# pathwaycom/pathway

Hardware: AMD Instinct MI355X
Metric: events/sec (whole node) on WordCount stream + p50 RAG query latency at fixed QPS (higher is better)
Workload: dtype int64/string-dict; 1 GPU; model=wordcount: stream -> groupby(word).count -> output deltas, global_batch=4000000, seq_len=1, parallelism=dp1 (shard exchange: RCCL all-to-all), vocab=50000, ingest=bytes, emitted_delta_rows=126750000, dict_misses=0

## Files before the change

pathway_amd/ops/__init__.py:

```python

from __future__ import annotations

import contextlib
import ctypes
import os
from typing import Sequence

import torch

_THIS = os.path.dirname(os.path.abspath(__file__))
_LIB_PATH = os.path.join(_THIS, "libpwhip.so")

_lib = None
_load_error: Exception | None = None


def _try_load():
    global _lib, _load_error
    if _lib is not None:
        return _lib
    try:
        if not os.path.exists(_LIB_PATH):
            from pathway_amd.ops import build as _build

# ... 467 lines not shown
    )
    oarr = (ctypes.c_void_p * max(nacc, 1))(
        *[ctypes.c_void_p(c.data_ptr()) for c in out_accs]
    )
    owarr = (ctypes.c_void_p * nw)(
        *[ctypes.c_void_p(w.data_ptr()) for w in out_words]
    )
    rc = lib.pw_seg_reduce_emit(
        warr,
        ctypes.c_int(nw),
        carr,
        ctypes.c_int(nacc),
        ctypes.c_int64(n),
        ctypes.c_void_p(bases.data_ptr()),
        owarr,
        ctypes.c_void_p(out_first.data_ptr()),
        oarr,
        ctypes.c_int64(nblocks),
        _stream_ptr(),
    )
    if rc != 0:
        raise RuntimeError(f"pw_seg_reduce_emit failed: hip error {rc}")
    return out_words, out_first, out_accs


def seg_reduce_gpu(
    k0: torch.Tensor, k1: torch.Tensor, contribs: Sequence[torch.Tensor]
) -> tuple[torch.Tensor, torch.Tensor, torch.Tensor, list]:
    out_words, out_first, out_accs = seg_reduce_words_gpu([k0, k1], contribs)
    return out_words[0], out_words[1], out_first, out_accs


_gc_temp_bytes: dict[int, int] = {}
_gc_temp_bytes_prefix: dict[int, int] = {}

_PW_GC_FULL_SORT = bool(os.environ.get("PW_GC_FULL_SORT"))

class _GcPathCounts(dict):

    bucket = 0

    def __getitem__(self, key):
        return self.bucket if key == "bucket" else dict.__getitem__(self, key)

    def __setitem__(self, key, value):
        if key == "bucket":
            self.bucket = value
        else:
            dict.__setitem__(self, key, value)


gc_path_counts = _GcPathCounts({"prefix": 0, "fallback": 0, "full": 0})

_gc_bucket_scope = False


@contextlib.contextmanager
def gc_bucket_scope(on: bool):
    global _gc_bucket_scope
    old, _gc_bucket_scope = _gc_bucket_scope, bool(on)
    try:
        yield
    finally:
        _gc_bucket_scope = old

gc_last_dirty_runs = 0

GC_BUCKET_MAX_LOAD = 0.5
GC_BUCKET_BITS = 8
GC_BUCKET_ROWS_FACTOR = 4
GC_BUCKET_MAX_PROBE = 128
GC_BUCKET_ROWS_FLOOR = 65536

_gc_bucket_caps: dict[int, int] = {}


def gc_bucket_capacity_limit(nacc: int) -> int:
    cap = _gc_bucket_caps.get(nacc)
    if cap is None:
        fn = require_lib().pw_gc_bucket_max_capacity
        fn.restype = ctypes.c_int64
        cap = int(fn(ctypes.c_int(nacc)))
        if cap < 2:
            raise RuntimeError("pw_gc_bucket_max_capacity failed")
        _gc_bucket_caps[nacc] = cap
    return cap


def gc_bucket_capacity(nacc: int) -> int:
    return min(gc_bucket_capacity_limit(nacc), 2048)


def gc_bucket_key_budget(nacc: int, bucket_bits: int = GC_BUCKET_BITS,
                         table_capacity: int | None = None) -> int:
    cap = table_capacity or gc_bucket_capacity(nacc)
    return (1 << bucket_bits) * int(GC_BUCKET_MAX_LOAD * cap)


def _gc_temp(lib, n: int, prefix: bool, dev) -> tuple[torch.Tensor, int]:
    cache = _gc_temp_bytes_prefix if prefix else _gc_temp_bytes
    tbytes = cache.get(n)
    if tbytes is None:
        fn = lib.pw_gc_temp_bytes_prefix if prefix else lib.pw_gc_temp_bytes
        fn.restype = ctypes.c_int64
        tbytes = int(fn(ctypes.c_int64(n)))
        if tbytes <= 0:
            raise RuntimeError("pw_gc_temp_bytes failed")
        cache[n] = tbytes
    return torch.empty(tbytes, dtype=torch.uint8, device=dev), tbytes


def _group_combine_two_sorts(keys_n2, contribs):
    k0, k1 = keys_n2[:, 0], keys_n2[:, 1]
    perm = torch.argsort(k1, stable=True)
    perm = perm.index_select(0, torch.argsort(k0.index_select(0, perm), stable=True))
    uk0, uk1, first_sorted, accs = seg_reduce_gpu(
        k0.index_select(0, perm),
        k1.index_select(0, perm),
        [c.index_select(0, perm) for c in contribs],
    )
    return uk0, uk1, perm.index_select(0, first_sorted), accs


def _group_combine_bucket(
    lib, keys_n2, contribs, bucket_bits, table_capacity, max_bucket_rows
):
    n = keys_n2.shape[0]
    dev = keys_n2.device
    nacc = len(contribs)
    nb = 1 << bucket_bits
    max_distinct = max(1, int(GC_BUCKET_MAX_LOAD * table_capacity))
    stream = _stream_ptr()
    temp, tbytes = _gc_temp(lib, n, True, dev)
    scratch32 = torch.empty((3, n), dtype=torch.int32, device=dev)
    staged = torch.empty((2 + max(nacc, 1), n), dtype=torch.int64, device=dev)
    bounds = torch.empty(2 * nb + 1, dtype=torch.int32, device=dev)
    base_ctl = torch.empty(nb + 3, dtype=torch.int64, device=dev)
    carr = (ctypes.c_void_p * max(nacc, 1))(
        *[ctypes.c_void_p(c.data_ptr()) for c in contribs]
    )
    sarr = (ctypes.c_void_p * max(nacc, 1))(
        *[ctypes.c_void_p(staged[2 + a].data_ptr()) for a in range(nacc)]
    )
    rc = lib.pw_gc_bucket_agg(
        ctypes.c_void_p(keys_n2.data_ptr()),
        ctypes.c_int64(n),
        ctypes.c_void_p(temp.data_ptr()),
        ctypes.c_int64(tbytes),
        ctypes.c_void_p(scratch32[0].data_ptr()),
        ctypes.c_void_p(scratch32[1].data_ptr()),
        ctypes.c_int(bucket_bits),
        ctypes.c_int64(table_capacity),
        ctypes.c_int64(max_distinct),
        ctypes.c_int64(max_bucket_rows),
        ctypes.c_int64(min(table_capacity, GC_BUCKET_MAX_PROBE)),
        carr,
        ctypes.c_int(nacc),
        ctypes.c_void_p(bounds.data_ptr()),
        ctypes.c_void_p(bounds[nb + 1 :].data_ptr()),
        ctypes.c_void_p(base_ctl.data_ptr()),
        ctypes.c_void_p(staged[0].data_ptr()),
        ctypes.c_void_p(staged[1].data_ptr()),
        ctypes.c_void_p(scratch32[2].data_ptr()),
        sarr,
        ctypes.c_void_p(base_ctl[nb + 1 :].data_ptr()),
        stream,
    )
    if rc != 0:
        raise RuntimeError(f"pw_gc_bucket_agg failed: hip error {rc}")
    total, overflow = base_ctl[nb + 1 :].tolist()
    if overflow:
        return None
    out_k = torch.empty((2, total), dtype=torch.int64, device=dev)
    out_first = torch.empty(total, dtype=torch.int64, device=dev)
    out_accs = torch.empty((max(nacc, 1), total), dtype=torch.int64, device=dev)
    oarr = (ctypes.c_void_p * max(nacc, 1))(
        *[ctypes.c_void_p(out_accs[a].data_ptr()) for a in range(nacc)]
    )
    rc = lib.pw_gc_bucket_compact(
        ctypes.c_void_p(base_ctl.data_ptr()),
        ctypes.c_void_p(bounds.data_ptr()),
        ctypes.c_int(bucket_bits),
        ctypes.c_int64(total),
        ctypes.c_void_p(staged[0].data_ptr()),
        ctypes.c_void_p(staged[1].data_ptr()),
        ctypes.c_void_p(scratch32[2].data_ptr()),
        sarr,
        ctypes.c_int(nacc),
        ctypes.c_void_p(out_k[0].data_ptr()),
        ctypes.c_void_p(out_k[1].data_ptr()),
        ctypes.c_void_p(out_first.data_ptr()),
        oarr,
        stream,
    )
    if rc != 0:
        raise RuntimeError(f"pw_gc_bucket_compact failed: hip error {rc}")
    return out_k[0], out_k[1], out_first, [out_accs[a] for a in range(nacc)]


def group_combine_gpu(
    keys_n2: torch.Tensor,
    contribs: Sequence[torch.Tensor],
    *,
    prefix_bits: int = 32,
    max_run: int = 2048,
    max_dirty: int = 65536,
    full_sort: bool = False,
    bucket: bool | None = None,
    bucket_bits: int = GC_BUCKET_BITS,
    table_capacity: int | None = None,
    max_bucket_rows: int | None = None,
) -> tuple[torch.Tensor, torch.Tensor, torch.Tensor, list]:
    global gc_last_dirty_runs
    lib = require_lib()
    n = keys_n2.shape[0]
    dev = keys_n2.device
    nacc = len(contribs)
    assert keys_n2.dim() == 2 and keys_n2.shape[1] == 2
    assert keys_n2.dtype == torch.int64
    assert 2 <= n < 2**32 and nacc <= 8
    assert 1 <= prefix_bits <= 32 and 2 <= max_run <= 3072
    assert 1 <= max_dirty < 2**32
    if keys_n2.stride() != (2, 1):
        keys_n2 = keys_n2.contiguous()
    contribs = [c.contiguous() for c in contribs]
    assert all(c.dtype == torch.int64 and c.shape == (n,) for c in contribs)
    if bucket is None:
        bucket = _gc_bucket_scope
    if bucket and not (full_sort or _PW_GC_FULL_SORT) and n < 2**32 - 1:
        assert 1 <= bucket_bits <= 16
        cap = table_capacity or gc_bucket_capacity(nacc)
        assert 2 <= cap <= gc_bucket_capacity_limit(nacc) and cap & (cap - 1) == 0
        if max_bucket_rows is None:
            even = -(-n // (1 << bucket_bits))
            max_bucket_rows = max(GC_BUCKET_ROWS_FACTOR * even, GC_BUCKET_ROWS_FLOOR)
        assert max_bucket_rows >= 1
        res = _group_combine_bucket(
            lib, keys_n2, contribs, bucket_bits, cap, max_bucket_rows
        )
        if res is not None:
            gc_path_counts["bucket"] += 1
            return res
    sorted_k = torch.empty((2, n), dtype=torch.int64, device=dev)
    perm32 = torch.empty(n, dtype=torch.int32, device=dev)
    nblocks = (n + 255) // 256
    block_counts = torch.empty(nblocks, dtype=torch.int32, device=dev)
    csum_ctrl = torch.empty(nblocks + 2, dtype=torch.int64, device=dev)
    csum = csum_ctrl[:nblocks]
    dirty_list = torch.empty(max_dirty, dtype=torch.int32, device=dev)
    stream = _stream_ptr()
    full_sort = full_sort or _PW_GC_FULL_SORT
    nseg = -1
    if not full_sort:
        temp, tbytes = _gc_temp(lib, n, True, dev)
        rc = lib.pw_gc_prefix_sort_count(
            ctypes.c_void_p(keys_n2.data_ptr()),
            ctypes.c_int64(n),
            ctypes.c_void_p(temp.data_ptr()),
            ctypes.c_int64(tbytes),
            ctypes.c_void_p(sorted_k[0].data_ptr()),
            ctypes.c_void_p(sorted_k[1].data_ptr()),
            ctypes.c_void_p(perm32.data_ptr()),
            ctypes.c_int(prefix_bits),
            ctypes.c_int64(max_run),
            ctypes.c_int64(max_dirty),
            ctypes.c_void_p(dirty_list.data_ptr()),
            ctypes.c_void_p(csum_ctrl[nblocks:].data_ptr()),
            ctypes.c_void_p(block_counts.data_ptr()),
            stream,
        )
        if rc != 0:
            raise RuntimeError(f"pw_gc_prefix_sort_count failed: hip error {rc}")
        torch.cumsum(block_counts, 0, dtype=torch.int64, out=csum)
        nseg, overflow, gc_last_dirty_runs = csum_ctrl[nblocks - 1 :].tolist()
        if overflow:
            nseg = -1
        else:
            gc_path_counts["prefix"] += 1
    if nseg < 0:
        temp, tbytes = _gc_temp(lib, n, False, dev)
        rc = lib.pw_gc_sort_count(
            ctypes.c_void_p(keys_n2.data_ptr()),
            ctypes.c_int64(n),
            ctypes.c_void_p(temp.data_ptr()),
            ctypes.c_int64(tbytes),
            ctypes.c_void_p(sorted_k[0].data_ptr()),
            ctypes.c_void_p(sorted_k[1].data_ptr()),
            ctypes.c_void_p(perm32.data_ptr()),
            ctypes.c_int(4),
            ctypes.c_int64(max_run),
            ctypes.c_int64(max_dirty),
            ctypes.c_void_p(dirty_list.data_ptr()),
            ctypes.c_void_p(csum_ctrl[nblocks:].data_ptr()),
            ctypes.c_void_p(block_counts.data_ptr()),
# ... 856 lines not shown
```

pathway_amd/ops/csrc/hip/pw_kernels.hip:

```cpp
#include <hip/hip_runtime.h>
#include <stdint.h>
#include <stdio.h>

#include <cstring>
#include <rocprim/rocprim.hpp>

#include "../xxhash_common.h"

#define PW_BLOCK 256
#define PW_MAX_GRID 2048

static inline int pw_grid(int64_t n) {
  int64_t g = (n + PW_BLOCK - 1) / PW_BLOCK;
  if (g > PW_MAX_GRID) g = PW_MAX_GRID;
  if (g < 1) g = 1;
  return (int)g;
}


struct WordPtrs {
  const uint64_t* p[20];
};

template <int W>
// ... 2406 lines not shown
                     s, (const long long*)keys, (const uint32_t*)perm32,
                     (long long*)k1_sorted, n, (unsigned long long*)ctrl);
  int64_t pairs = n / 2 + 1;
  int64_t rblocks = (pairs + PW_BLOCK - 1) / PW_BLOCK;
  for (int p = 0; p < passes; ++p)
    hipLaunchKernelGGL(k_gc_sort_repair, dim3((uint32_t)rblocks),
                       dim3(PW_BLOCK), 0, s, (const long long*)k0_sorted,
                       (long long*)k1_sorted, (uint32_t*)perm32, n, p & 1);
  return gc_repair_count(k0_sorted, k1_sorted, perm32, n, 0, max_run,
                         max_dirty, dirty_list, ctrl, block_counts, s);
}

extern "C" int64_t pw_gc_temp_bytes_prefix(int64_t n) {
  size_t bytes = 0;
  if (n <= 0 || n >= ((int64_t)1 << 32)) return 0;
  if (gc_sort_prefix(nullptr, bytes, nullptr, nullptr, nullptr, n, 32, 0) !=
      hipSuccess)
    return 0;
  return (int64_t)bytes;
}

extern "C" int pw_gc_prefix_sort_count(const void* keys, int64_t n, void* temp,
                                       int64_t temp_bytes, void* k0_sorted,
                                       void* k1_sorted, void* perm32,
                                       int prefix_bits, int64_t max_run,
                                       int64_t max_dirty, void* dirty_list,
                                       void* ctrl, void* block_counts,
                                       void* stream) {
  if (n < 2 || n >= ((int64_t)1 << 32)) return 1;
  if (prefix_bits < 1 || prefix_bits > 32) return 1;
  if (max_run < 2 || max_run > PW_GC_MAX_RUN_LIMIT) return 1;
  if (max_dirty < 1 || max_dirty >= ((int64_t)1 << 32)) return 1;
  hipStream_t s = (hipStream_t)stream;
  size_t tb = (size_t)temp_bytes;
  hipError_t e = gc_sort_prefix(temp, tb, (const long long*)keys,
                                (uint32_t*)k1_sorted, (uint32_t*)perm32, n,
                                prefix_bits, s);
  if (e != hipSuccess) return (int)e;
  hipLaunchKernelGGL(k_gc_gather_k01, dim3(2 * PW_MAX_GRID), dim3(PW_BLOCK), 0,
                     s, (const long long*)keys, (const uint32_t*)perm32,
                     (long long*)k0_sorted, (long long*)k1_sorted, n,
                     (unsigned long long*)ctrl);
  return gc_repair_count(k0_sorted, k1_sorted, perm32, n, 64 - prefix_bits,
                         max_run, max_dirty, dirty_list, ctrl, block_counts,
                         s);
}


#define PW_GC_BK_THREADS 1024
#define PW_GC_BK_UNPUB 0xFFFFFFFFu
#define PW_GC_BK_LDS_MAX 61440
#define PW_GC_BK_UNROLL 4

__global__ void k_gc_bucket_bounds(const uint32_t* __restrict__ prefix_sorted,
                                   int64_t n, uint32_t nb,
                                   uint32_t* bucket_start,
                                   unsigned long long* ctl) {
  uint32_t b = blockIdx.x * blockDim.x + threadIdx.x;
  if (b == 0) {
    ctl[0] = 0;
    ctl[1] = 0;
  }
  if (b > nb) return;
  int64_t lo = 0, hi = n;
  while (lo < hi) {
    int64_t mid = (lo + hi) >> 1;
    if (prefix_sorted[mid] < b) lo = mid + 1;
    else hi = mid;
  }
  bucket_start[b] = (uint32_t)lo;
}

__device__ __forceinline__ uint32_t gc_bk_hash(unsigned long long w0,
                                               long long w1, int lg_cap) {
  uint32_t h = (uint32_t)w0 ^ (uint32_t)(w0 >> 29) ^
               ((uint32_t)w1 * 0x9E3779B1u);
  return (h * 0x85EBCA6Bu) >> (32 - lg_cap);
}

__global__ __launch_bounds__(PW_GC_BK_THREADS) void k_gc_bucket_agg(
    const long long* __restrict__ keys, const uint32_t* __restrict__ perm32,
    const uint32_t* __restrict__ bucket_start, AccPtrs contribs, int nacc,
    int bucket_bits, uint32_t cap, int lg_cap, uint32_t max_distinct,
    uint32_t max_rows, uint32_t max_probe, long long* st_k0, long long* st_k1,
    uint32_t* st_first, AccPtrsMut st_accs, uint32_t* bucket_uniques,
    unsigned long long* ctl) {
  extern __shared__ unsigned long long gcb_lds[];
  unsigned long long* t0 = gcb_lds;
  long long* t1 = (long long*)(t0 + cap);
  unsigned long long* tacc = (unsigned long long*)(t1 + cap);
  uint32_t* tfirst = (uint32_t*)(tacc + (size_t)nacc * cap);
  uint16_t* list = (uint16_t*)(tfirst + cap);
  __shared__ uint32_t s_cnt, s_claims, s_ovf;

  const uint32_t b = blockIdx.x;
  const uint32_t tid = threadIdx.x;
  const uint32_t beg = bucket_start[b], end = bucket_start[b + 1];
  const uint32_t rows = end - beg;
  if (rows == 0 || rows > max_rows) {
    if (tid == 0) {
      bucket_uniques[b] = 0;
      if (rows) ctl[1] = 1;
    }
    return;
  }
  const uint32_t mask = cap - 1;
  const unsigned long long empty =
      (unsigned long long)((b ^ 1u) ^ (1u << (bucket_bits - 1)))
      << (64 - bucket_bits);
  for (uint32_t s = tid; s < cap; s += PW_GC_BK_THREADS) {
    t0[s] = empty;
    tfirst[s] = PW_GC_BK_UNPUB;
    for (int a = 0; a < nacc; ++a) tacc[(size_t)a * cap + s] = 0;
  }
  if (tid == 0) s_cnt = 0, s_claims = 0, s_ovf = 0;
  __syncthreads();

  const long long* c0 = contribs.p[0];
  for (int64_t base = (int64_t)beg + tid; base < (int64_t)end;
       base += (int64_t)PW_GC_BK_UNROLL * PW_GC_BK_THREADS) {
    uint32_t row[PW_GC_BK_UNROLL];
    unsigned long long k0[PW_GC_BK_UNROLL];
    long long k1[PW_GC_BK_UNROLL];
    unsigned long long v0[PW_GC_BK_UNROLL];
#pragma unroll
    for (int q = 0; q < PW_GC_BK_UNROLL; ++q) {
      int64_t i = base + (int64_t)q * PW_GC_BK_THREADS;
      row[q] = i < (int64_t)end ? perm32[i] : PW_GC_BK_UNPUB;
    }
#pragma unroll
    for (int q = 0; q < PW_GC_BK_UNROLL; ++q) {
      if (row[q] == PW_GC_BK_UNPUB) continue;
      k0[q] = (unsigned long long)keys[2 * (size_t)row[q]];
      k1[q] = keys[2 * (size_t)row[q] + 1];
      v0[q] = nacc > 0 ? (unsigned long long)c0[row[q]] : 0ULL;
    }
#pragma unroll
    for (int q = 0; q < PW_GC_BK_UNROLL; ++q) {
      if (row[q] == PW_GC_BK_UNPUB) continue;
      if (__hip_atomic_load(&s_ovf, __ATOMIC_RELAXED,
                            __HIP_MEMORY_SCOPE_WORKGROUP))
        break;
      const unsigned long long key0 = k0[q];
      const long long key1 = k1[q];
      uint32_t slot = gc_bk_hash(key0, key1, lg_cap);
      bool done = false;
      for (uint32_t tries = 0; tries < max_probe; ++tries) {
        bool match;
        const unsigned long long cur = __hip_atomic_load(
            &t0[slot], __ATOMIC_ACQUIRE, __HIP_MEMORY_SCOPE_WORKGROUP);
        if (cur != empty) {
          match = cur == key0 && t1[slot] == key1;
          if (match) atomicMin(&tfirst[slot], row[q]);
        } else {
          const uint32_t f = atomicCAS(&tfirst[slot], PW_GC_BK_UNPUB, row[q]);
          match = f == PW_GC_BK_UNPUB;
          if (match) {
            if (atomicAdd(&s_claims, 1u) >= max_distinct) s_ovf = 1;
            t1[slot] = key1;
            __hip_atomic_store(&t0[slot], key0, __ATOMIC_RELEASE,
                               __HIP_MEMORY_SCOPE_WORKGROUP);
          } else {
            match = (unsigned long long)keys[2 * (size_t)f] == key0 &&
                    keys[2 * (size_t)f + 1] == key1;
            if (match) atomicMin(&tfirst[slot], row[q]);
          }
        }
        if (match) {
          if (nacc > 0) atomicAdd(&tacc[slot], v0[q]);
          for (int a = 1; a < nacc; ++a)
            atomicAdd(&tacc[(size_t)a * cap + slot],
                      (unsigned long long)contribs.p[a][row[q]]);
          done = true;
          break;
        }
        slot = (slot + 1) & mask;
      }
      if (!done) s_ovf = 1;
    }
  }
  __syncthreads();

  for (uint32_t s = tid; s < cap; s += PW_GC_BK_THREADS)
    if (tfirst[s] != PW_GC_BK_UNPUB) list[atomicAdd(&s_cnt, 1u)] = (uint16_t)s;
  __syncthreads();
  const uint32_t cnt = s_cnt;
  if (s_ovf || cnt > max_distinct) {
    if (tid == 0) {
      bucket_uniques[b] = 0;
      ctl[1] = 1;
    }
    return;
  }

  for (uint32_t t = tid; t < cnt; t += PW_GC_BK_THREADS) {
    const uint32_t sl = list[t];
    const long long a0 = (long long)t0[sl], a1 = t1[sl];
    uint32_t rank = 0;
    for (uint32_t u = 0; u < cnt; ++u) {
      const uint32_t su = list[u];
      const long long b0 = (long long)t0[su];
      rank += (b0 < a0 || (b0 == a0 && t1[su] < a1)) ? 1u : 0u;
    }
    const size_t o = (size_t)beg + rank;
    st_k0[o] = a0;
    st_k1[o] = a1;
    st_first[o] = tfirst[sl];
    for (int a = 0; a < nacc; ++a)
      st_accs.p[a][o] = (long long)tacc[(size_t)a * cap + sl];
  }
  if (tid == 0) bucket_uniques[b] = cnt;
}

__global__ void k_gc_bucket_scan(const uint32_t* __restrict__ uniq,
                                 uint32_t nb, long long* base,
                                 unsigned long long* ctl) {
  __shared__ long long part[PW_BLOCK];
  const uint32_t tid = threadIdx.x;
  const uint32_t chunk = (nb + PW_BLOCK - 1) / PW_BLOCK;
  const uint32_t lo = tid * chunk < nb ? tid * chunk : nb;
  const uint32_t hi = lo + chunk < nb ? lo + chunk : nb;
  long long sum = 0;
  for (uint32_t i = lo; i < hi; ++i) sum += uniq[i];
  part[tid] = sum;
  __syncthreads();
// ... 42 lines not shown
static inline size_t gc_bk_entry_bytes(int nacc) {
  return 8 + 8 + 8 * (size_t)nacc + 4 + 2;
}

extern "C" int64_t pw_gc_bucket_max_capacity(int nacc) {
  if (nacc < 0 || nacc > 8) return 0;
  int64_t cap = 1;
  while ((size_t)(2 * cap) * gc_bk_entry_bytes(nacc) <= PW_GC_BK_LDS_MAX)
    cap *= 2;
  return cap;
}

extern "C" int pw_gc_bucket_agg(const void* keys, int64_t n, void* temp,
                                int64_t temp_bytes, void* prefix_scratch,
                                void* perm32, int bucket_bits,
                                int64_t table_capacity, int64_t max_distinct,
                                int64_t max_bucket_rows, int64_t max_probe,
                                const void** contrib_ptrs, int nacc,
                                void* bucket_start, void* bucket_uniques,
                                void* base, void* st_k0, void* st_k1,
                                void* st_first, void** st_acc_ptrs, void* ctl,
                                void* stream) {
  if (n < 2 || n >= ((int64_t)1 << 32) - 1) return 1;
  if (bucket_bits < 1 || bucket_bits > 16) return 1;
  if (nacc < 0 || nacc > 8) return 1;
  if (table_capacity < 2 || table_capacity > 32768 ||
      (table_capacity & (table_capacity - 1)))
    return 1;
  size_t lds = (size_t)table_capacity * gc_bk_entry_bytes(nacc);
  if (lds > PW_GC_BK_LDS_MAX) return 1;
  if (max_distinct < 1 || max_distinct > table_capacity) return 1;
  if (max_bucket_rows < 1 || max_probe < 1) return 1;
  if (max_bucket_rows > 0xFFFFFFFFLL) max_bucket_rows = 0xFFFFFFFFLL;
  if (max_probe > table_capacity) max_probe = table_capacity;
  int lg_cap = 0;
  while (((int64_t)1 << lg_cap) < table_capacity) ++lg_cap;
  hipStream_t s = (hipStream_t)stream;
  size_t tb = (size_t)temp_bytes;
  hipError_t e = gc_sort_prefix(temp, tb, (const long long*)keys,
                                (uint32_t*)prefix_scratch, (uint32_t*)perm32,
                                n, bucket_bits, s);
  if (e != hipSuccess) return (int)e;
  AccPtrs cp;
  AccPtrsMut sp;
  for (int a = 0; a < 8; ++a) {
    cp.p[a] = a < nacc ? (const long long*)contrib_ptrs[a] : nullptr;
    sp.p[a] = a < nacc ? (long long*)st_acc_ptrs[a] : nullptr;
  }
  uint32_t nb = 1u << bucket_bits;
  hipLaunchKernelGGL(k_gc_bucket_bounds,
                     dim3((nb + 1 + PW_BLOCK - 1) / PW_BLOCK), dim3(PW_BLOCK),
                     0, s, (const uint32_t*)prefix_scratch, n, nb,
                     (uint32_t*)bucket_start, (unsigned long long*)ctl);
  hipLaunchKernelGGL(k_gc_bucket_agg, dim3(nb), dim3(PW_GC_BK_THREADS), lds, s,
                     (const long long*)keys, (const uint32_t*)perm32,
                     (const uint32_t*)bucket_start, cp, nacc, bucket_bits,
                     (uint32_t)table_capacity, lg_cap, (uint32_t)max_distinct,
                     (uint32_t)max_bucket_rows, (uint32_t)max_probe,
                     (long long*)st_k0, (long long*)st_k1, (uint32_t*)st_first,
                     sp, (uint32_t*)bucket_uniques, (unsigned long long*)ctl);
  hipLaunchKernelGGL(k_gc_bucket_scan, dim3(1), dim3(PW_BLOCK), 0, s,
                     (const uint32_t*)bucket_uniques, nb, (long long*)base,
                     (unsigned long long*)ctl);
  return (int)hipGetLastError();
}

extern "C" int pw_gc_bucket_compact(const void* base, const void* bucket_start,
                                    int bucket_bits, int64_t total,
                                    const void* st_k0, const void* st_k1,
                                    const void* st_first,
                                    const void** st_acc_ptrs, int nacc,
                                    void* out_k0, void* out_k1,
                                    void* out_first, void** out_acc_ptrs,
                                    void* stream) {
  if (bucket_bits < 1 || bucket_bits > 16 || nacc < 0 || nacc > 8) return 1;
  if (total < 1) return 0;
  AccPtrs sp;
  AccPtrsMut op;
  for (int a = 0; a < 8; ++a) {
    sp.p[a] = a < nacc ? (const long long*)st_acc_ptrs[a] : nullptr;
    op.p[a] = a < nacc ? (long long*)out_acc_ptrs[a] : nullptr;
  }
  int64_t nblocks = (total + PW_BLOCK - 1) / PW_BLOCK;
  hipLaunchKernelGGL(k_gc_bucket_compact, dim3((uint32_t)nblocks),
                     dim3(PW_BLOCK), 0, (hipStream_t)stream,
                     (const long long*)base, (const uint32_t*)bucket_start,
                     1u << bucket_bits, total, (const long long*)st_k0,
                     (const long long*)st_k1, (const uint32_t*)st_first, sp,
                     nacc, (long long*)out_k0, (long long*)out_k1,
                     (long long*)out_first, op);
  return (int)hipGetLastError();
}

extern "C" int pw_gc_emit(const void* k0_sorted, const void* k1_sorted,
                          const void* perm32, const void** contrib_ptrs,
                          int nacc, int64_t n, const void* block_csum,
                          void* out_k0, void* out_k1, void* out_first,
                          void** out_acc_ptrs, void* stream) {
  if (nacc < 0 || nacc > 8 || n < 1) return 1;
  AccPtrs cp;
  AccPtrsMut op;
  for (int a = 0; a < nacc; ++a) {
    cp.p[a] = (const long long*)contrib_ptrs[a];
    op.p[a] = (long long*)out_acc_ptrs[a];
  }
  hipStream_t s = (hipStream_t)stream;
  int64_t nblocks = (n + PW_BLOCK - 1) / PW_BLOCK;
  hipLaunchKernelGGL(k_gc_emit, dim3((uint32_t)nblocks), dim3(PW_BLOCK), 0, s,
                     (const long long*)k0_sorted, (const long long*)k1_sorted,
// ... 604 lines not shown
```

profiles/gc_bucket_sweep.py:

```python

import json
import statistics
import time

import torch

from pathway_amd import ops

N, VOCAB, REPS = 4_000_000, 50_000, 20


def timed(keys, contribs, **kw):
    before = {k: ops.gc_path_counts[k] for k in ("prefix", "fallback", "bucket")}
    ts = []
    for i in range(REPS + 3):
        torch.cuda.synchronize()
        t0 = time.perf_counter()
        ops.group_combine_gpu(keys, contribs, **kw)
        torch.cuda.synchronize()
        if i >= 3:
            ts.append((time.perf_counter() - t0) * 1e3)
    path = [k for k, v in before.items() if ops.gc_path_counts[k] != v]
    return round(statistics.median(ts), 4), "+".join(path)


def main():
    g = torch.Generator(device="cpu").manual_seed(1)
    table = torch.randint(-(1 << 63), (1 << 63) - 1, (VOCAB, 2), generator=g)
    keys = table[torch.randint(0, VOCAB, (N,), generator=g)].cuda()
    ones = [torch.ones(N, dtype=torch.int64, device="cuda")]
    ms, path = timed(keys, ones, bucket=False)
    print(json.dumps({"case": "50k distinct", "bucket": False, "ms": ms, "path": path}))
    for bits in (6, 8, 9, 10, 12):
        for cap in (512, 1024, 2048):
            ms, path = timed(keys, ones, bucket=True, bucket_bits=bits, table_capacity=cap)
            print(json.dumps({"case": "50k distinct", "bucket_bits": bits,
                              "table_capacity": cap, "ms": ms, "path": path}))
    distinct = torch.randint(-(1 << 63), (1 << 63) - 1, (N, 2), generator=g).cuda()
    for on in (False, True):
        ms, path = timed(distinct, ones, bucket=on)
        print(json.dumps({"case": "all distinct", "bucket": on, "ms": ms, "path": path}))


if __name__ == "__main__":
    main()
```

Baseline: 3.522 billion events/s.

## Partition rows by key bucket before hash aggregation instead of gathering via sort

Adds a three-kernel radix partition (per-tile histogram, scan, LDS-staged scatter) that physically moves keys, row ids and contributions into bucket-contiguous order, so the bucket aggregation kernel reads them with coalesced loads. Before this, the path sorted a prefix permutation and then gathered keys and contributions indirectly. The partition path becomes the default for bucket_bits <= 8. It costs extra staging memory for the partitioned copies and may clone the keys to get 16-byte alignment. It only runs when the bucket scope is enabled.

After: 3.792 billion events/s (median of 6 runs). +7.7%, better.

```diff
diff --git a/pathway_amd/ops/__init__.py b/pathway_amd/ops/__init__.py
--- a/pathway_amd/ops/__init__.py
+++ b/pathway_amd/ops/__init__.py
@@ -543,6 +543,12 @@
 
 gc_path_counts = _GcPathCounts({"prefix": 0, "fallback": 0, "full": 0})
 
+_PW_NO_GC_PARTITION = bool(os.environ.get("PW_NO_GC_PARTITION"))
+_PW_GC_PART_DIRECT = bool(os.environ.get("PW_GC_PART_DIRECT"))
+gc_bucket_layout_counts = {"partition": 0, "gather": 0}
+GC_PART_TILE = 8192
+GC_PART_MAX_BITS = 8
+
 _gc_bucket_scope = False
 
 
@@ -613,8 +619,77 @@
     return uk0, uk1, perm.index_select(0, first_sorted), accs
 
 
+def _gc_part_hist_entries(lib, n: int, bucket_bits: int) -> int:
+    fn = lib.pw_gc_part_hist_entries
+    fn.restype = ctypes.c_int64
+    entries = int(fn(ctypes.c_int64(n), ctypes.c_int(bucket_bits)))
+    if entries <= 0:
+        raise RuntimeError("pw_gc_part_hist_entries failed")
+    tile = lib.pw_gc_part_tile
+    tile.restype = ctypes.c_int64
+    assert int(tile()) == GC_PART_TILE
+    return entries
+
+
+def _gc_aligned_keys(keys_n2: torch.Tensor) -> torch.Tensor:
+    return keys_n2.clone() if keys_n2.data_ptr() % 16 else keys_n2
+
+
+def gc_partition_gpu(
+    keys_n2: torch.Tensor, contribs: Sequence[torch.Tensor], bucket_bits: int
+) -> tuple[torch.Tensor, torch.Tensor, torch.Tensor, list]:
+    lib = require_lib()
+    n = keys_n2.shape[0]
+    dev = keys_n2.device
+    nacc = len(contribs)
+    assert keys_n2.dim() == 2 and keys_n2.shape[1] == 2
+    assert keys_n2.dtype == torch.int64
+    assert 2 <= n < 2**32 - 1 and nacc <= 8 and 1 <= bucket_bits <= 8
+    if keys_n2.stride() != (2, 1):
+        keys_n2 = keys_n2.contiguous()
+    keys_n2 = _gc_aligned_keys(keys_n2)
+    contribs = [c.contiguous() for c in contribs]
+    assert all(c.dtype == torch.int64 and c.shape == (n,) for c in contribs)
+    nb = 1 << bucket_bits
+    hist = _gc_part_hist_entries(lib, n, bucket_bits)
+    part64 = torch.empty((2 + nacc, n), dtype=torch.int64, device=dev)
+    scratch32 = torch.empty(hist + n + nb + 1, dtype=torch.int32, device=dev)
+    ctl = torch.empty(2, dtype=torch.int64, device=dev)
+    carr = (ctypes.c_void_p * max(nacc, 1))(
+        *[ctypes.c_void_p(c.data_ptr()) for c in contribs]
+    )
+    parr = (ctypes.c_void_p * max(nacc, 1))(
+        *[ctypes.c_void_p(part64[2 + a].data_ptr()) for a in range(nacc)]
+    )
+    rc = lib.pw_gc_partition(
+        ctypes.c_void_p(keys_n2.data_ptr()),
+        ctypes.c_int64(n),
+        ctypes.c_int(bucket_bits),
+        carr,
+        ctypes.c_int(nacc),
+        ctypes.c_void_p(scratch32.data_ptr()),
+        ctypes.c_void_p(part64.data_ptr()),
+        ctypes.c_void_p(scratch32[hist:].data_ptr()),
+        parr,
+        ctypes.c_void_p(scratch32[hist + n :].data_ptr()),
+        ctypes.c_void_p(ctl.data_ptr()),
+        ctypes.c_int(int(_PW_GC_PART_DIRECT)),
+        _stream_ptr(),
+    )
+    if rc != 0:
+        raise RuntimeError(f"pw_gc_partition failed: hip error {rc}")
+    u32 = lambda t: t.to(torch.int64) & 0xFFFFFFFF
+    return (
+        u32(scratch32[hist + n :]),
+        part64[:2].reshape(n, 2),
+        u32(scratch32[hist : hist + n]),
+        [part64[2 + a] for a in range(nacc)],
+    )
+
+
 def _group_combine_bucket(
-    lib, keys_n2, contribs, bucket_bits, table_capacity, max_bucket_rows
+    lib, keys_n2, contribs, bucket_bits, table_capacity, max_bucket_rows,
+    partition=False,
 ):
     n = keys_n2.shape[0]
     dev = keys_n2.device
@@ -622,43 +697,86 @@
     nb = 1 << bucket_bits
     max_distinct = max(1, int(GC_BUCKET_MAX_LOAD * table_capacity))
     stream = _stream_ptr()
-    temp, tbytes = _gc_temp(lib, n, True, dev)
-    scratch32 = torch.empty((3, n), dtype=torch.int32, device=dev)
-    staged = torch.empty((2 + max(nacc, 1), n), dtype=torch.int64, device=dev)
     bounds = torch.empty(2 * nb + 1, dtype=torch.int32, device=dev)
     base_ctl = torch.empty(nb + 3, dtype=torch.int64, device=dev)
     carr = (ctypes.c_void_p * max(nacc, 1))(
         *[ctypes.c_void_p(c.data_ptr()) for c in contribs]
     )
+    if partition:
+        keys_n2 = _gc_aligned_keys(keys_n2)
+        hist = _gc_part_hist_entries(lib, n, bucket_bits)
+        scratch32 = torch.empty(hist + 2 * n, dtype=torch.int32, device=dev)
+        st_first = scratch32[hist + n :]
+        staged = torch.empty(
+            (2 + nacc + 2 + max(nacc, 1), n), dtype=torch.int64, device=dev
+        )
+        st0 = 2 + nacc
+        parr = (ctypes.c_void_p * max(nacc, 1))(
+            *[ctypes.c_void_p(staged[2 + a].data_ptr()) for a in range(nacc)]
+        )
+    else:
+        temp, tbytes = _gc_temp(lib, n, True, dev)
+        scratch32 = torch.empty((3, n), dtype=torch.int32, device=dev)
+        st_first = scratch32[2]
+        staged = torch.empty((2 + max(nacc, 1), n), dtype=torch.int64, device=dev)
+        st0 = 0
     sarr = (ctypes.c_void_p * max(nacc, 1))(
-        *[ctypes.c_void_p(staged[2 + a].data_ptr()) for a in range(nacc)]
-    )
-    rc = lib.pw_gc_bucket_agg(
-        ctypes.c_void_p(keys_n2.data_ptr()),
-        ctypes.c_int64(n),
-        ctypes.c_void_p(temp.data_ptr()),
-        ctypes.c_int64(tbytes),
-        ctypes.c_void_p(scratch32[0].data_ptr()),
-        ctypes.c_void_p(scratch32[1].data_ptr()),
-        ctypes.c_int(bucket_bits),
-        ctypes.c_int64(table_capacity),
-        ctypes.c_int64(max_distinct),
-        ctypes.c_int64(max_bucket_rows),
-        ctypes.c_int64(min(table_capacity, GC_BUCKET_MAX_PROBE)),
-        carr,
-        ctypes.c_int(nacc),
-        ctypes.c_void_p(bounds.data_ptr()),
-        ctypes.c_void_p(bounds[nb + 1 :].data_ptr()),
-        ctypes.c_void_p(base_ctl.data_ptr()),
-        ctypes.c_void_p(staged[0].data_ptr()),
-        ctypes.c_void_p(staged[1].data_ptr()),
-        ctypes.c_void_p(scratch32[2].data_ptr()),
-        sarr,
-        ctypes.c_void_p(base_ctl[nb + 1 :].data_ptr()),
-        stream,
-    )
-    if rc != 0:
-        raise RuntimeError(f"pw_gc_bucket_agg failed: hip error {rc}")
+        *[ctypes.c_void_p(staged[st0 + 2 + a].data_ptr()) for a in range(nacc)]
+    )
+    if partition:
+        rc = lib.pw_gc_bucket_part_agg(
+            ctypes.c_void_p(keys_n2.data_ptr()),
+            ctypes.c_int64(n),
+            ctypes.c_int(bucket_bits),
+            ctypes.c_int64(table_capacity),
+            ctypes.c_int64(max_distinct),
+            ctypes.c_int64(max_bucket_rows),
+            ctypes.c_int64(min(table_capacity, GC_BUCKET_MAX_PROBE)),
+            carr,
+            ctypes.c_int(nacc),
+            ctypes.c_void_p(scratch32.data_ptr()),
+            ctypes.c_void_p(staged.data_ptr()),
+            ctypes.c_void_p(scratch32[hist:].data_ptr()),
+            parr,
+            ctypes.c_void_p(bounds.data_ptr()),
+            ctypes.c_void_p(bounds[nb + 1 :].data_ptr()),
+            ctypes.c_void_p(base_ctl.data_ptr()),
+            ctypes.c_void_p(staged[st0].data_ptr()),
+            ctypes.c_void_p(staged[st0 + 1].data_ptr()),
+            ctypes.c_void_p(st_first.data_ptr()),
+            sarr,
+            ctypes.c_void_p(base_ctl[nb + 1 :].data_ptr()),
+            ctypes.c_int(int(_PW_GC_PART_DIRECT)),
+            stream,
+        )
+    else:
+        rc = lib.pw_gc_bucket_agg(
+            ctypes.c_void_p(keys_n2.data_ptr()),
+            ctypes.c_int64(n),
+            ctypes.c_void_p(temp.data_ptr()),
+            ctypes.c_int64(tbytes),
+            ctypes.c_void_p(scratch32[0].data_ptr()),
+            ctypes.c_void_p(scratch32[1].data_ptr()),
+            ctypes.c_int(bucket_bits),
+            ctypes.c_int64(table_capacity),
+            ctypes.c_int64(max_distinct),
+            ctypes.c_int64(max_bucket_rows),
+            ctypes.c_int64(min(table_capacity, GC_BUCKET_MAX_PROBE)),
+            carr,
+            ctypes.c_int(nacc),
+            ctypes.c_void_p(bounds.data_ptr()),
+            ctypes.c_void_p(bounds[nb + 1 :].data_ptr()),
+            ctypes.c_void_p(base_ctl.data_ptr()),
+            ctypes.c_void_p(staged[0].data_ptr()),
+            ctypes.c_void_p(staged[1].data_ptr()),
+            ctypes.c_void_p(st_first.data_ptr()),
+            sarr,
+            ctypes.c_void_p(base_ctl[nb + 1 :].data_ptr()),
+            stream,
+        )
+    if rc != 0:
+        fn = "pw_gc_bucket_part_agg" if partition else "pw_gc_bucket_agg"
+        raise RuntimeError(f"{fn} failed: hip error {rc}")
     total, overflow = base_ctl[nb + 1 :].tolist()
     if overflow:
         return None
@@ -673,9 +791,9 @@
         ctypes.c_void_p(bounds.data_ptr()),
         ctypes.c_int(bucket_bits),
         ctypes.c_int64(total),
-        ctypes.c_void_p(staged[0].data_ptr()),
-        ctypes.c_void_p(staged[1].data_ptr()),
-        ctypes.c_void_p(scratch32[2].data_ptr()),
+        ctypes.c_void_p(staged[st0].data_ptr()),
+        ctypes.c_void_p(staged[st0 + 1].data_ptr()),
+        ctypes.c_void_p(st_first.data_ptr()),
         sarr,
         ctypes.c_int(nacc),
         ctypes.c_void_p(out_k[0].data_ptr()),
@@ -701,6 +819,7 @@
     bucket_bits: int = GC_BUCKET_BITS,
     table_capacity: int | None = None,
     max_bucket_rows: int | None = None,
+    partition: bool | None = None,
 ) -> tuple[torch.Tensor, torch.Tensor, torch.Tensor, list]:
     global gc_last_dirty_runs
     lib = require_lib()
@@ -726,11 +845,15 @@
             even = -(-n // (1 << bucket_bits))
             max_bucket_rows = max(GC_BUCKET_ROWS_FACTOR * even, GC_BUCKET_ROWS_FLOOR)
         assert max_bucket_rows >= 1
+        if partition is None:
+            partition = not _PW_NO_GC_PARTITION
+        partition = bool(partition) and bucket_bits <= GC_PART_MAX_BITS
         res = _group_combine_bucket(
-            lib, keys_n2, contribs, bucket_bits, cap, max_bucket_rows
+            lib, keys_n2, contribs, bucket_bits, cap, max_bucket_rows, partition
         )
         if res is not None:
             gc_path_counts["bucket"] += 1
+            gc_bucket_layout_counts["partition" if partition else "gather"] += 1
             return res
     sorted_k = torch.empty((2, n), dtype=torch.int64, device=dev)
     perm32 = torch.empty(n, dtype=torch.int32, device=dev)
diff --git a/pathway_amd/ops/csrc/hip/pw_kernels.hip b/pathway_amd/ops/csrc/hip/pw_kernels.hip
--- a/pathway_amd/ops/csrc/hip/pw_kernels.hip
+++ b/pathway_amd/ops/csrc/hip/pw_kernels.hip
@@ -2482,6 +2482,243 @@
 #define PW_GC_BK_LDS_MAX 61440
 #define PW_GC_BK_UNROLL 4
 
+#define PW_GC_PT_THREADS 1024
+#define PW_GC_PT_TILE 8192
+#define PW_GC_PT_ROWS (PW_GC_PT_TILE / PW_GC_PT_THREADS)
+#define PW_GC_PT_SUB 2048
+#define PW_GC_PT_SCAN_RANGES 32
+
+__device__ __forceinline__ uint32_t gc_pt_bucket(unsigned long long w0,
+                                                 int drop) {
+  return ((uint32_t)(w0 >> 32) ^ 0x80000000u) >> drop;
+}
+
+static inline uint32_t gc_pt_stride(uint32_t nb) { return nb < 8 ? 8 : nb; }
+
+__host__ __device__ static inline uint32_t gc_pt_chunk(uint32_t nblk) {
+  return (nblk + PW_GC_PT_SCAN_RANGES - 1) / PW_GC_PT_SCAN_RANGES;
+}
+
+__global__ __launch_bounds__(PW_GC_PT_THREADS) void k_gc_part_count(
+    const long long* __restrict__ keys, int64_t n, int drop, uint32_t nbp,
+    uint32_t* __restrict__ block_hist) {
+  __shared__ uint32_t h[256];
+  const uint32_t tid = threadIdx.x;
+  if (tid < 256) h[tid] = 0;
+  __syncthreads();
+  const int64_t base = (int64_t)blockIdx.x * PW_GC_PT_TILE + tid;
+  unsigned long long w[PW_GC_PT_ROWS];
+#pragma unroll
+  for (int q = 0; q < PW_GC_PT_ROWS; ++q) {
+    const int64_t i = base + (int64_t)q * PW_GC_PT_THREADS;
+    w[q] = i < n ? (unsigned long long)keys[2 * (size_t)i] : 0ULL;
+  }
+#pragma unroll
+  for (int q = 0; q < PW_GC_PT_ROWS; ++q) {
+    const int64_t i = base + (int64_t)q * PW_GC_PT_THREADS;
+    if (i < n) atomicAdd(&h[gc_pt_bucket(w[q], drop)], 1u);
+  }
+  __syncthreads();
+  if (tid < nbp) block_hist[(size_t)blockIdx.x * nbp + tid] = h[tid];
+}
+
+__global__ __launch_bounds__(PW_GC_PT_THREADS) void k_gc_part_scan(
+    const uint32_t* __restrict__ block_hist, uint32_t nblk, uint32_t nb,
+    uint32_t nbp, int64_t n, uint32_t* __restrict__ bucket_start,
+    uint32_t* __restrict__ range_base, unsigned long long* ctl) {
+  __shared__ uint32_t part[PW_GC_PT_SCAN_RANGES][256];
+  __shared__ uint32_t sc[256];
+  const uint32_t tid = threadIdx.x;
+  const uint32_t no = nbp / 8;
+  const uint32_t tb = tid % no, tr = tid / no;
+  const bool active = tr < PW_GC_PT_SCAN_RANGES;
+  const uint32_t chunk = gc_pt_chunk(nblk);
+  const uint32_t lo = tr * chunk < nblk ? tr * chunk : nblk;
+  const uint32_t hi = lo + chunk < nblk ? lo + chunk : nblk;
+  const uint4* h4 = (const uint4*)block_hist;
+  if (tid == 0) {
+    ctl[0] = 0;
+    ctl[1] = 0;
+  }
+  if (active) {
+    uint4 s = make_uint4(0, 0, 0, 0), t = make_uint4(0, 0, 0, 0);
+#pragma unroll 8
+    for (uint32_t blk = lo; blk < hi; ++blk) {
+      const uint4 v = h4[((size_t)blk * no + tb) * 2];
+      const uint4 w = h4[((size_t)blk * no + tb) * 2 + 1];
+      s.x += v.x, s.y += v.y, s.z += v.z, s.w += v.w;
+      t.x += w.x, t.y += w.y, t.z += w.z, t.w += w.w;
+    }
+    uint32_t* p = &part[tr][8 * tb];
+    p[0] = s.x, p[1] = s.y, p[2] = s.z, p[3] = s.w;
+    p[4] = t.x, p[5] = t.y, p[6] = t.z, p[7] = t.w;
+  }
+  __syncthreads();
+  uint32_t tot = 0;
+  if (tid < nbp) {
+    for (int r = 0; r < PW_GC_PT_SCAN_RANGES; ++r) {
+      const uint32_t v = part[r][tid];
+      part[r][tid] = tot;
+      tot += v;
+    }
+  }
+  if (tid < 256) sc[tid] = tot;
+  __syncthreads();
+  for (uint32_t off = 1; off < 256; off <<= 1) {
+    const uint32_t v = (tid < 256 && tid >= off) ? sc[tid - off] : 0;
+    __syncthreads();
+    if (tid < 256) sc[tid] += v;
+    __syncthreads();
+  }
+  if (tid < 256) {
+    const uint32_t ex = sc[tid] - tot;
+    sc[tid] = ex;
+    if (tid < nb) bucket_start[tid] = ex;
+  }
+  if (tid == 0) bucket_start[nb] = (uint32_t)n;
+  __syncthreads();
+  for (uint32_t e = tid; e < PW_GC_PT_SCAN_RANGES * nbp; e += PW_GC_PT_THREADS)
+    range_base[e] = sc[e % nbp] + part[e / nbp][e % nbp];
+}
+
+template <bool STAGED>
+__global__ __launch_bounds__(PW_GC_PT_THREADS) void k_gc_part_scatter(
+    const long long* __restrict__ keys, AccPtrs contribs, int nacc, int64_t n,
+    int drop, uint32_t nbp, const uint32_t* __restrict__ block_hist,
+    const uint32_t* __restrict__ range_base, long long* __restrict__ part_keys,
+    uint32_t* __restrict__ part_row, AccPtrsMut part_acc) {
+  __shared__ uint32_t cur[256];
+  const uint32_t tid = threadIdx.x;
+  const ulonglong2* __restrict__ k2 = (const ulonglong2*)keys;
+  ulonglong2* __restrict__ o2 = (ulonglong2*)part_keys;
+  const long long* __restrict__ c0 = contribs.p[0];
+  const int64_t tile = (int64_t)blockIdx.x * PW_GC_PT_TILE;
+  if (tid < nbp) {
+    const uint32_t chunk = gc_pt_chunk(gridDim.x);
+    const uint32_t r = blockIdx.x / chunk;
+    uint32_t v = range_base[r * nbp + tid];
+    for (uint32_t blk = r * chunk; blk < blockIdx.x; ++blk)
+      v += block_hist[(size_t)blk * nbp + tid];
+    cur[tid] = v;
+  }
+  if constexpr (!STAGED) {
+    __syncthreads();
+    for (int g = 0; g < PW_GC_PT_ROWS; g += 4) {
+      ulonglong2 kv[4];
+      long long v0[4];
+#pragma unroll
+      for (int q = 0; q < 4; ++q) {
+        const int64_t i = tile + (int64_t)(g + q) * PW_GC_PT_THREADS + tid;
+        if (i < n) {
+          kv[q] = k2[i];
+          v0[q] = nacc > 0 ? c0[i] : 0;
+        }
+      }
+#pragma unroll
+      for (int q = 0; q < 4; ++q) {
+        const int64_t i = tile + (int64_t)(g + q) * PW_GC_PT_THREADS + tid;
+        if (i >= n) continue;
+        const uint32_t dst = atomicAdd(&cur[gc_pt_bucket(kv[q].x, drop)], 1u);
+        o2[dst] = kv[q];
+        part_row[dst] = (uint32_t)i;
+        if (nacc > 0) part_acc.p[0][dst] = v0[q];
+        for (int a = 1; a < nacc; ++a) part_acc.p[a][dst] = contribs.p[a][i];
+      }
+    }
+  } else {
+    constexpr int SQ = PW_GC_PT_SUB / PW_GC_PT_THREADS;
+    __shared__ ulonglong2 bufk[PW_GC_PT_SUB];
+    __shared__ long long bufa[PW_GC_PT_SUB];
+    __shared__ uint32_t bufr[PW_GC_PT_SUB];
+    __shared__ uint8_t bkt[PW_GC_PT_SUB];
+    __shared__ uint32_t cnt[256], lstart[256], delta[256], wtot[4];
+    for (int64_t sbase = tile; sbase < tile + PW_GC_PT_TILE && sbase < n;
+         sbase += PW_GC_PT_SUB) {
+      const uint32_t m =
+          n - sbase < PW_GC_PT_SUB ? (uint32_t)(n - sbase) : PW_GC_PT_SUB;
+      if (tid < 256) cnt[tid] = 0;
+      __syncthreads();
+      ulonglong2 kv[SQ];
+      long long v0[SQ];
+      uint32_t bk[SQ], lp[SQ];
+#pragma unroll
+      for (int q = 0; q < SQ; ++q) {
+        const uint32_t j = q * PW_GC_PT_THREADS + tid;
+        if (j < m) {
+          kv[q] = k2[sbase + j];
+          v0[q] = nacc > 0 ? c0[sbase + j] : 0;
+        }
+      }
+#pragma unroll
+      for (int q = 0; q < SQ; ++q) {
+        const uint32_t j = q * PW_GC_PT_THREADS + tid;
+        if (j < m) {
+          bk[q] = gc_pt_bucket(kv[q].x, drop);
+          lp[q] = atomicAdd(&cnt[bk[q]], 1u);
+        }
+      }
+      __syncthreads();
+      uint32_t c = 0, inc = 0;
+      if (tid < 256) {
+        c = cnt[tid];
+        inc = c;
+#pragma unroll
+        for (int d = 1; d < 64; d <<= 1) {
+          const uint32_t up = __shfl_up(inc, d);
+          if ((tid & 63) >= (uint32_t)d) inc += up;
+        }
+        if ((tid & 63) == 63) wtot[tid >> 6] = inc;
+      }
+      __syncthreads();
+      if (tid < 256) {
+        uint32_t off = 0;
+        for (uint32_t w = 0; w < (tid >> 6); ++w) off += wtot[w];
+        const uint32_t ex = off + inc - c;
+        lstart[tid] = ex;
+        delta[tid] = cur[tid] - ex;
+        cur[tid] += c;
+      }
+      __syncthreads();
+#pragma unroll
+      for (int q = 0; q < SQ; ++q) {
+        const uint32_t j = q * PW_GC_PT_THREADS + tid;
+        if (j < m) {
+          lp[q] += lstart[bk[q]];
+          bufk[lp[q]] = kv[q];
+          bufr[lp[q]] = (uint32_t)(sbase + j);
+          bkt[lp[q]] = (uint8_t)bk[q];
+          if (nacc > 0) bufa[lp[q]] = v0[q];
+        }
+      }
+      __syncthreads();
+#pragma unroll
+      for (int q = 0; q < SQ; ++q) {
+        const uint32_t j = q * PW_GC_PT_THREADS + tid;
+        if (j < m) {
+          const uint32_t dst = delta[bkt[j]] + j;
+          o2[dst] = bufk[j];
+          part_row[dst] = bufr[j];
+          if (nacc > 0) part_acc.p[0][dst] = bufa[j];
+        }
+      }
+      for (int a = 1; a < nacc; ++a) {
+        __syncthreads();
+#pragma unroll
+        for (int q = 0; q < SQ; ++q) {
+          const uint32_t j = q * PW_GC_PT_THREADS + tid;
+          if (j < m) bufa[lp[q]] = contribs.p[a][sbase + j];
+        }
+        __syncthreads();
+#pragma unroll
+        for (int q = 0; q < SQ; ++q) {
+          const uint32_t j = q * PW_GC_PT_THREADS + tid;
+          if (j < m) part_acc.p[a][delta[bkt[j]] + j] = bufa[j];
+        }
+      }
+    }
+  }
+}
+
 __global__ void k_gc_bucket_bounds(const uint32_t* __restrict__ prefix_sorted,
                                    int64_t n, uint32_t nb,
                                    uint32_t* bucket_start,
@@ -2508,8 +2745,10 @@
   return (h * 0x85EBCA6Bu) >> (32 - lg_cap);
 }
 
+template <bool PART, int NV>
 __global__ __launch_bounds__(PW_GC_BK_THREADS) void k_gc_bucket_agg(
     const long long* __restrict__ keys, const uint32_t* __restrict__ perm32,
+    const long long* __restrict__ part_keys,
     const uint32_t* __restrict__ bucket_start, AccPtrs contribs, int nacc,
     int bucket_bits, uint32_t cap, int lg_cap, uint32_t max_distinct,
     uint32_t max_rows, uint32_t max_probe, long long* st_k0, long long* st_k1,
@@ -2552,7 +2791,7 @@
     uint32_t row[PW_GC_BK_UNROLL];
     unsigned long long k0[PW_GC_BK_UNROLL];
     long long k1[PW_GC_BK_UNROLL];
-    unsigned long long v0[PW_GC_BK_UNROLL];
+    unsigned long long v[PW_GC_BK_UNROLL][NV];
 #pragma unroll
     for (int q = 0; q < PW_GC_BK_UNROLL; ++q) {
       int64_t i = base + (int64_t)q * PW_GC_BK_THREADS;
@@ -2561,9 +2800,19 @@
 #pragma unroll
     for (int q = 0; q < PW_GC_BK_UNROLL; ++q) {
       if (row[q] == PW_GC_BK_UNPUB) continue;
-      k0[q] = (unsigned long long)keys[2 * (size_t)row[q]];
-      k1[q] = keys[2 * (size_t)row[q] + 1];
-      v0[q] = nacc > 0 ? (unsigned long long)c0[row[q]] : 0ULL;
+      if constexpr (PART) {
+        const int64_t i = base + (int64_t)q * PW_GC_BK_THREADS;
+        const ulonglong2 kv = ((const ulonglong2*)part_keys)[i];
+        k0[q] = kv.x;
+        k1[q] = (long long)kv.y;
+#pragma unroll
+        for (int a = 0; a < NV; ++a)
+          v[q][a] = a < nacc ? (unsigned long long)contribs.p[a][i] : 0ULL;
+      } else {
+        k0[q] = (unsigned long long)keys[2 * (size_t)row[q]];
+        k1[q] = keys[2 * (size_t)row[q] + 1];
+        v[q][0] = nacc > 0 ? (unsigned long long)c0[row[q]] : 0ULL;
+      }
     }
 #pragma unroll
     for (int q = 0; q < PW_GC_BK_UNROLL; ++q) {
@@ -2597,10 +2846,16 @@
           }
         }
         if (match) {
-          if (nacc > 0) atomicAdd(&tacc[slot], v0[q]);
-          for (int a = 1; a < nacc; ++a)
-            atomicAdd(&tacc[(size_t)a * cap + slot],
-                      (unsigned long long)contribs.p[a][row[q]]);
+          if (nacc > 0) atomicAdd(&tacc[slot], v[q][0]);
+          if constexpr (PART) {
+#pragma unroll
+            for (int a = 1; a < NV; ++a)
+              if (a < nacc) atomicAdd(&tacc[(size_t)a * cap + slot], v[q][a]);
+          } else {
+            for (int a = 1; a < nacc; ++a)
+              atomicAdd(&tacc[(size_t)a * cap + slot],
+                        (unsigned long long)contribs.p[a][row[q]]);
+          }
           done = true;
           break;
         }
@@ -2749,9 +3004,127 @@
                      dim3((nb + 1 + PW_BLOCK - 1) / PW_BLOCK), dim3(PW_BLOCK),
                      0, s, (const uint32_t*)prefix_scratch, n, nb,
                      (uint32_t*)bucket_start, (unsigned long long*)ctl);
-  hipLaunchKernelGGL(k_gc_bucket_agg, dim3(nb), dim3(PW_GC_BK_THREADS), lds, s,
-                     (const long long*)keys, (const uint32_t*)perm32,
+  hipLaunchKernelGGL((k_gc_bucket_agg<false, 1>), dim3(nb),
+                     dim3(PW_GC_BK_THREADS), lds, s, (const long long*)keys,
+                     (const uint32_t*)perm32, (const long long*)nullptr,
                      (const uint32_t*)bucket_start, cp, nacc, bucket_bits,
+                     (uint32_t)table_capacity, lg_cap, (uint32_t)max_distinct,
+                     (uint32_t)max_bucket_rows, (uint32_t)max_probe,
+                     (long long*)st_k0, (long long*)st_k1, (uint32_t*)st_first,
+                     sp, (uint32_t*)bucket_uniques, (unsigned long long*)ctl);
+  hipLaunchKernelGGL(k_gc_bucket_scan, dim3(1), dim3(PW_BLOCK), 0, s,
+                     (const uint32_t*)bucket_uniques, nb, (long long*)base,
+                     (unsigned long long*)ctl);
+  return (int)hipGetLastError();
+}
+
+extern "C" int64_t pw_gc_part_tile() { return PW_GC_PT_TILE; }
+
+extern "C" int64_t pw_gc_part_hist_entries(int64_t n, int bucket_bits) {
+  if (n < 2 || n >= ((int64_t)1 << 32) - 1) return 0;
+  if (bucket_bits < 1 || bucket_bits > 8) return 0;
+  int64_t nblk = (n + PW_GC_PT_TILE - 1) / PW_GC_PT_TILE;
+  return (nblk + PW_GC_PT_SCAN_RANGES) *
+         (int64_t)gc_pt_stride(1u << bucket_bits);
+}
+
+static void gc_partition_launch(const long long* keys, int64_t n,
+                                int bucket_bits, const AccPtrs& cp, int nacc,
+                                uint32_t* block_hist, long long* part_keys,
+                                uint32_t* part_row, const AccPtrsMut& pp,
+                                uint32_t* bucket_start,
+                                unsigned long long* ctl, int direct,
+                                hipStream_t s) {
+  const uint32_t nb = 1u << bucket_bits, nbp = gc_pt_stride(nb);
+  const uint32_t nblk = (uint32_t)((n + PW_GC_PT_TILE - 1) / PW_GC_PT_TILE);
+  const int drop = 32 - bucket_bits;
+  uint32_t* range_base = block_hist + (size_t)nblk * nbp;
+  hipLaunchKernelGGL(k_gc_part_count, dim3(nblk), dim3(PW_GC_PT_THREADS), 0, s,
+                     keys, n, drop, nbp, block_hist);
+  hipLaunchKernelGGL(k_gc_part_scan, dim3(1), dim3(PW_GC_PT_THREADS), 0, s,
+                     (const uint32_t*)block_hist, nblk, nb, nbp, n,
+                     bucket_start, range_base, ctl);
+  if (direct)
+    hipLaunchKernelGGL(k_gc_part_scatter<false>, dim3(nblk),
+                       dim3(PW_GC_PT_THREADS), 0, s, keys, cp, nacc, n, drop,
+                       nbp, (const uint32_t*)block_hist,
+                       (const uint32_t*)range_base, part_keys, part_row, pp);
+  else
+    hipLaunchKernelGGL(k_gc_part_scatter<true>, dim3(nblk),
+                       dim3(PW_GC_PT_THREADS), 0, s, keys, cp, nacc, n, drop,
+                       nbp, (const uint32_t*)block_hist,
+                       (const uint32_t*)range_base, part_keys, part_row, pp);
+}
+
+static bool gc_partition_args_ok(const void* keys, int64_t n, int bucket_bits,
+                                 int nacc, const void* block_hist,
+                                 const void* part_keys) {
+  if (n < 2 || n >= ((int64_t)1 << 32) - 1) return false;
+  if (bucket_bits < 1 || bucket_bits > 8) return false;
+  if (nacc < 0 || nacc > 8) return false;
+  return ((uintptr_t)keys | (uintptr_t)block_hist | (uintptr_t)part_keys) % 16 == 0;
+}
+
+extern "C" int pw_gc_partition(const void* keys, int64_t n, int bucket_bits,
+                               const void** contrib_ptrs, int nacc,
+                               void* block_hist, void* part_keys,
+                               void* part_row, void** part_acc_ptrs,
+                               void* bucket_start, void* ctl, int direct,
+                               void* stream) {
+  if (!gc_partition_args_ok(keys, n, bucket_bits, nacc, block_hist, part_keys))
+    return 1;
+  AccPtrs cp;
+  AccPtrsMut pp;
+  for (int a = 0; a < 8; ++a) {
+    cp.p[a] = a < nacc ? (const long long*)contrib_ptrs[a] : nullptr;
+    pp.p[a] = a < nacc ? (long long*)part_acc_ptrs[a] : nullptr;
+  }
+  gc_partition_launch((const long long*)keys, n, bucket_bits, cp, nacc,
+                      (uint32_t*)block_hist, (long long*)part_keys,
+                      (uint32_t*)part_row, pp, (uint32_t*)bucket_start,
+                      (unsigned long long*)ctl, direct, (hipStream_t)stream);
+  return (int)hipGetLastError();
+}
+
+extern "C" int pw_gc_bucket_part_agg(
+    const void* keys, int64_t n, int bucket_bits, int64_t table_capacity,
+    int64_t max_distinct, int64_t max_bucket_rows, int64_t max_probe,
+    const void** contrib_ptrs, int nacc, void* block_hist, void* part_keys,
+    void* part_row, void** part_acc_ptrs, void* bucket_start,
+    void* bucket_uniques, void* base, void* st_k0, void* st_k1, void* st_first,
+    void** st_acc_ptrs, void* ctl, int direct, void* stream) {
+  if (!gc_partition_args_ok(keys, n, bucket_bits, nacc, block_hist, part_keys))
+    return 1;
+  if (table_capacity < 2 || table_capacity > 32768 ||
+      (table_capacity & (table_capacity - 1)))
+    return 1;
+  size_t lds = (size_t)table_capacity * gc_bk_entry_bytes(nacc);
+  if (lds > PW_GC_BK_LDS_MAX) return 1;
+  if (max_distinct < 1 || max_distinct > table_capacity) return 1;
+  if (max_bucket_rows < 1 || max_probe < 1) return 1;
+  if (max_bucket_rows > 0xFFFFFFFFLL) max_bucket_rows = 0xFFFFFFFFLL;
+  if (max_probe > table_capacity) max_probe = table_capacity;
+  int lg_cap = 0;
+  while (((int64_t)1 << lg_cap) < table_capacity) ++lg_cap;
+  hipStream_t s = (hipStream_t)stream;
+  AccPtrs cp, pc;
+  AccPtrsMut pp, sp;
+  for (int a = 0; a < 8; ++a) {
+    cp.p[a] = a < nacc ? (const long long*)contrib_ptrs[a] : nullptr;
+    pp.p[a] = a < nacc ? (long long*)part_acc_ptrs[a] : nullptr;
+    pc.p[a] = pp.p[a];
+    sp.p[a] = a < nacc ? (long long*)st_acc_ptrs[a] : nullptr;
+  }
+  gc_partition_launch((const long long*)keys, n, bucket_bits, cp, nacc,
+                      (uint32_t*)block_hist, (long long*)part_keys,
+                      (uint32_t*)part_row, pp, (uint32_t*)bucket_start,
+                      (unsigned long long*)ctl, direct, s);
+  const uint32_t nb = 1u << bucket_bits;
+  auto agg = nacc <= 1 ? k_gc_bucket_agg<true, 1> : k_gc_bucket_agg<true, 8>;
+  hipLaunchKernelGGL(agg, dim3(nb), dim3(PW_GC_BK_THREADS), lds, s,
+                     (const long long*)keys, (const uint32_t*)part_row,
+                     (const long long*)part_keys,
+                     (const uint32_t*)bucket_start, pc, nacc, bucket_bits,
                      (uint32_t)table_capacity, lg_cap, (uint32_t)max_distinct,
                      (uint32_t)max_bucket_rows, (uint32_t)max_probe,
                      (long long*)st_k0, (long long*)st_k1, (uint32_t*)st_first,
diff --git a/profiles/gc_bucket_sweep.py b/profiles/gc_bucket_sweep.py
--- a/profiles/gc_bucket_sweep.py
+++ b/profiles/gc_bucket_sweep.py
@@ -33,9 +33,13 @@
     print(json.dumps({"case": "50k distinct", "bucket": False, "ms": ms, "path": path}))
     for bits in (6, 8, 9, 10, 12):
         for cap in (512, 1024, 2048):
-            ms, path = timed(keys, ones, bucket=True, bucket_bits=bits, table_capacity=cap)
-            print(json.dumps({"case": "50k distinct", "bucket_bits": bits,
-                              "table_capacity": cap, "ms": ms, "path": path}))
+            for part in ((True, False) if bits <= ops.GC_PART_MAX_BITS else (False,)):
+                ms, path = timed(keys, ones, bucket=True, bucket_bits=bits,
+                                 table_capacity=cap, partition=part)
+                print(json.dumps({"case": "50k distinct", "bucket_bits": bits,
+                                  "table_capacity": cap,
+                                  "layout": "partition" if part else "gather",
+                                  "ms": ms, "path": path}))
     distinct = torch.randint(-(1 << 63), (1 << 63) - 1, (N, 2), generator=g).cuda()
     for on in (False, True):
         ms, path = timed(distinct, ones, bucket=on)
```
